# Griffan/VerifyBamID

Measured on AMD Instinct MI355X. Metric: llk_evals_per_sec, higher is better.
Workload: dtype f64; 1 GPU; synthetic pileup 100000 markers x depth 30, --NumPC 4 (BASELINE.json configs[2] shape); parallelism=1 GPU, rccl_world_size=1, launched_by=single process, reads=2999230, active_markers=100000, distinct_codes=42, device=gfx950:sramecc+:xnack-

## Files before the change

### verifybamid_amd/csrc/kernel_debug.h

```cpp
#ifndef VB2_KERNEL_DEBUG_H_
#define VB2_KERNEL_DEBUG_H_

#ifndef VB2_ABLATE
#define VB2_ABLATE 0
#endif
#ifndef VB2_FLAG_RELEASE
#define VB2_FLAG_RELEASE 1
#endif
#ifndef VB2_SOFT_PROLOGUE
#define VB2_SOFT_PROLOGUE 1
#endif
#ifndef VB2_CTRL_PRIO
#define VB2_CTRL_PRIO 3
#endif
#ifndef VB2_SPLIT_FAST
#define VB2_SPLIT_FAST 3
#endif
#ifndef VB2_STAMP_ROUND
#define VB2_STAMP_ROUND 0
#endif

namespace vb2 {
constexpr int kAblNoMap = 1, kAblNoTable = 2, kAblNoItems = 4, kAblNoReads = 8, kAblNoEpi = 16, kAblNoSignal = 32, kAblNoMul = 64, kAblNoRowLoads = 128;
constexpr int kAblate = VB2_ABLATE;
constexpr int kSplitFast = VB2_SPLIT_FAST;
}

#ifdef VB2_WITH_STAMPS
#define VB2_STAMPS_OF(L) ((L).stamps)
#else
#define VB2_STAMPS_OF(L) (static_cast<unsigned long long*>(nullptr))
#endif

#ifdef VB2_ITEM_PROF
#define VB2_IP_T(var) const unsigned long long var = __builtin_readcyclecounter()
#define VB2_IP_USE(x) asm volatile("" ::"v"(x))
#else
#define VB2_IP_T(var)
#define VB2_IP_USE(x)
#endif

#endif
```

### verifybamid_amd/csrc/llk_kernels.hip

```cpp
#include "llk_kernels.h"

#include <hip/hip_runtime.h>
#include <link.h>

#include "kernel_debug.h"
#include "tile_sched.h"
#include "tunables.h"
#ifndef VB2_SIMD_DEAL
#define VB2_SIMD_DEAL 1
#endif

#include <algorithm>
#include <atomic>
#include <cstring>
#include <type_traits>
#include <vector>

namespace vb2 {

__device__ __forceinline__ void pair_of(int p, int& g1, int& g2)
{
    g1 = p >> 1;
    const int lo = p & 1;
    g2 = lo + (lo >= g1 ? 1 : 0);
// ... 247 lines not shown
}
__device__ __forceinline__ int lane_of(int m, int g)
{
    const int idx = ((g & 1) << 2) + (m >> 2);
    const int q = (0x74216530u >> (4 * idx)) & 7;
    return ((g >> 1) << 5) + (q << 2) + (m & 3);
}

__device__ __forceinline__ int lane_xchg_i32(int x, int off, int partner)
{
    if (off == 1) return __builtin_amdgcn_update_dpp(0, x, 0xB1, 0xf, 0xf, true);
    if (off == 2) return __builtin_amdgcn_update_dpp(0, x, 0x4E, 0xf, 0xf, true);
    if (off == 4) {
        const int a = __builtin_amdgcn_update_dpp(0, x, 0x124, 0xf, 0x5, false);
        return __builtin_amdgcn_update_dpp(a, x, 0x12C, 0xf, 0xa, false);
    }
    return __shfl(x, partner, 64);
}
__device__ __forceinline__ double lane_xchg_f64(double x, int off, int partner)
{
    if (off == 1 || off == 2 || off == 4)
        return __hiloint2double(lane_xchg_i32(__double2hiint(x), off, partner), lane_xchg_i32(__double2loint(x), off, partner));
    return __shfl(x, partner, 64);
}

template <int MODE> struct Geom { static constexpr int kMaxWaves = 16, kBlocksPerCU = 1, kWavesPerSimd = 4; };
template <int MODE> struct ModeNp { static constexpr int value = MODE == 2 ? 8 : MODE == 4 ? 1 : MODE == 5 ? 2 : 4; };

struct InlinePoints {
    int count;
    double v[kInlinePointDoubles];
};

struct NoHook {
    __device__ bool on_block() const { return false; }
    __device__ bool mine() const { return false; }
    __device__ void run() {}
    __device__ bool keep_etab() const { return false; }
    __device__ bool prim_in_lds() const { return false; }
    __device__ bool keep_prim() const { return false; }
    __device__ double* sum_stage() const { return nullptr; }
    __device__ uint32_t cache_rec() const { return 0u; }
    __device__ unsigned int* sync_word() const { return nullptr; }
    __device__ bool collect_only() const { return false; }
    __device__ bool no_collect() const { return false; }
};
__host__ __device__ __forceinline__ bool eval_is_dynamic(const DeviceLayout& L, uint32_t nblk, int nwave, int ngrp)
{
    const uint32_t max_tiles_blk = owned_most(L.pd ? 1 : 0, (uint32_t)L.num_mt, nblk);
    return max_tiles_blk * (uint32_t)ngrp <= (uint32_t)(L.dyn_limit * nwave);
}

template <int MODE, bool W16 = false, class Hook = NoHook, bool STREAM = false, int QUEUE = -1, int KSEL = 0,
          bool LCACHE = false, int ESH = 8, bool PD = false, int SPLIT = 0>
__device__ __forceinline__ void
eval_body(const DeviceLayout& L, const double* ip_v, const int ip_count, const double* __restrict__ points, int num_valid,
          double* __restrict__ partials, double* __restrict__ llk_out,
          unsigned int* __restrict__ ticket, unsigned long long* __restrict__ done_flag,
          unsigned long long done_seq, const uint32_t blk, const uint32_t nblk,
          unsigned int* __restrict__ batch_done, unsigned int batch_active, const int ngrp_in,
          const unsigned long long tag, const Schedule sch, const bool coherent_points = false,
          const int tid_in = -1, const double* lds_rows = nullptr ,
          Hook hook = Hook())
{
    extern __shared__ __attribute__((aligned(16))) double lds[];
    static_assert(MODE >= 2 && MODE <= 5, "wave shapes 2..5");
    static_assert(!PD || ESH == 8, "probability-domain contexts have no exp table");
    static_assert(!(PD && W16) || ((MODE == 4 || MODE == 5) && STREAM), "8-bit step lists: cohort steps of one and two points");
    static_assert(!SPLIT || (PD && MODE == 2 && QUEUE == 1 && !STREAM && !LCACHE), "split launches: the 8-point shape on the queue");
    constexpr int OSH = PD ? 1 : 0;
    constexpr bool ONEGRP = MODE != 2 || STREAM;
    constexpr int KAF = KSEL > 0 ? 0 : -1;
    constexpr int BTL = MODE == 4 ? 1 : 2;
    constexpr int TPW = MODE == 3 ? 2 : (MODE == 4 || MODE == 5) ? 4 : 1;
    constexpr int SLOTS = 4 / TPW;
    constexpr int NP = SLOTS * BTL;
    const int row_bytes = MODE == 2 ? kRowBytesWide : L.row_bytes;
    const int RS = row_bytes >> 3;
    const int nrow = L.num_code + 1;
    const int nthread = blockDim.x;
    const int nwave = nthread >> 6;
    const int k = KSEL > 0 ? KSEL : L.num_pc;
    const int stride = 2 * k + 1;
    constexpr int NVS = SPLIT ? SPLIT : 1;
    const int g_per = SPLIT ? (ngrp_in + NVS - 1) / NVS : ngrp_in;
    const int g_lo = SPLIT ? (int)(blk % (uint32_t)NVS) * g_per : 0;
    const int ngrp = ONEGRP ? 1 : SPLIT ? (ngrp_in - g_lo < g_per ? ngrp_in - g_lo : g_per) : ngrp_in;
    const int p_off = g_lo * NP;
    const uint32_t vstep = SPLIT ? nblk / (uint32_t)NVS : 0u, vb0 = SPLIT ? blk / (uint32_t)NVS : blk;
    const double* const known_af_p = KAF == 0 ? nullptr : L.known_af;
    const int NPT = NP * ngrp;
    constexpr int kEtabCopies = (1 << ESH) / 8, kEtabDoubles = PD ? 0 : 64 * kEtabCopies;
    constexpr int kLtabDoubles = PD ? 0 : kLogTabDoubles;
    double* etab = lds;
    double* ltab = lds + kEtabDoubles;
    double* tab = ltab + kLtabDoubles;
    double* red = tab + ngrp * nrow * RS;
    unsigned int* queue = reinterpret_cast<unsigned int*>(red + NVS * NPT);
    double* pts = red + NVS * NPT + 2;
    double* ptq = pts + (size_t)NPT * stride + ((NPT * stride) & 1);
    const size_t prim_off = (size_t)(ptq - lds) + (size_t)NPT * 2 * k;
    double2* prim_lds = reinterpret_cast<double2*>(lds + prim_off + (prim_off & 1));
    double* tile_llk = reinterpret_cast<double*>(prim_lds + L.num_prim);

    const int tid = tid_in >= 0 ? tid_in : (int)threadIdx.x;
    const int lane = tid & 63;
    const int wave = __builtin_amdgcn_readfirstlane(tid >> 6);
    int m, g4;
    lane_map(lane, m, g4);
    const int g = g4 & (SLOTS - 1);
    const int half = TPW == 1 ? 0 : g4 / SLOTS;
    const bool stamp_this = VB2_STAMP_ROUND == 0 || (unsigned)(tag & 0xffffffffull) == (unsigned)VB2_STAMP_ROUND;
#ifdef VB2_ITEM_PROF
    unsigned long long* stamps = nullptr;
#else
    unsigned long long* stamps = (VB2_STAMPS_OF(L) && stamp_this) ? VB2_STAMPS_OF(L) + (size_t)blk * 8 : nullptr;
#endif
    if (stamps && tid == 0) { stamps[0] = wall_clock64(); stamps[4] = 0; }
    if constexpr (SPLIT != 0) {
        if (stamps && tid == 0 && blk != 0u && blk != 20u && blk != 21u) {
            unsigned int xcc;
            asm volatile("s_getreg_b32 %0, hwreg(HW_REG_XCC_ID)" : "=s"(xcc));
            stamps[7] = 1ull + (xcc & 15u);
        }
    }

    const bool collect_only = hook.collect_only();
    if (collect_only && hook.mine()) hook.run();
    if (!collect_only) {
    const bool hook_blk = hook.on_block(), hook_mine = hook.mine();
    unsigned int* const soft_word = PD ? hook.sync_word() : nullptr;
    const bool soft = hook_blk && soft_word != nullptr;
    if (soft && hook_mine) hook.run();
    const int ptid = !soft ? tid : hook_mine ? 0x3fffffff : tid - 64, pnthread = soft ? nthread - 64 : nthread;
    unsigned int soft_gen = 0;
    auto prologue_sync = [&]() {
        if (!soft) { __syncthreads(); return; }
        if (hook_mine) return;
        soft_gen += (unsigned int)(nwave - 1);
        if (lane == 0) __hip_atomic_fetch_add(soft_word, 1u, __ATOMIC_RELAXED, __HIP_MEMORY_SCOPE_WORKGROUP);
        while (__hip_atomic_load(soft_word, __ATOMIC_RELAXED, __HIP_MEMORY_SCOPE_WORKGROUP) < soft_gen) __builtin_amdgcn_s_sleep(1);
        asm volatile("" ::: "memory");
    };
    constexpr bool SPLIT_EARLY = SPLIT != 0 && (kSplitFast & 1) != 0;
    constexpr int kTabSide = 3;
    const int ntab_split = (kAblate & kAblNoTable) ? 0 : (PD ? L.num_prim - L.num_pair : L.num_prim) * 6 * NP;
    auto table_inputs = [&](int e, int g0, double2& rec_o, double* al_o) {
        const int pi = e / (6 * NP);
        const int bb = (e - pi * (6 * NP)) / 6;
        rec_o = L.prim[pi];
#pragma unroll
        for (int u = 0; u < kTabSide; ++u) {
            const int ge = g0 + u < ngrp ? g0 + u : ngrp - 1;
            const int b = ge * NP + bb;
            const int idx = (p_off + b < num_valid ? p_off + b : num_valid - 1) * stride + 2 * k;
            al_o[u] = (kAblate & kAblNoMap) ? 0.01 * (double)(1 + idx % 7) : points[idx];
        }
    };
    double2 tin_rec = make_double2(0.0, 0.0);
    double tin_al[kTabSide] = {0.0, 0.0, 0.0};
    if constexpr (SPLIT_EARLY)
        if (ptid < ntab_split) table_inputs(ptid, 0, tin_rec, tin_al);
    if (ptid == 0) *queue = (unsigned int)(nwave - (hook_blk ? 1 : 0));
    for (int e = ptid; e < NPT * stride; e += pnthread) {
        const int b = e / stride;
        const int src = p_off + b < num_valid ? p_off + b : num_valid - 1;
        const int idx = src * stride + (e - b * stride);
        const double v = (kAblate & kAblNoMap) ? 0.01 * (double)(1 + idx % 7)
                         : lds_rows ? lds_rows[idx]
                         : ip_count > 0 ? ip_v[idx]
                         : coherent_points ? __hip_atomic_load(&points[idx], __ATOMIC_RELAXED, __HIP_MEMORY_SCOPE_AGENT)
                                           : points[idx];
        pts[e] = v;
        const int c = e - b * stride;
        if (c < 2 * k) ptq[((b / BTL) * 2 * k + c) * BTL + (b % BTL)] = v;
    }
    if (!PD && !hook.keep_etab() && tid < kLogTabDoubles / 2)
        reinterpret_cast<double2*>(ltab)[tid] = kLogTabRows[tid];
    if (!PD && !hook.keep_etab())
        for (int jb = 2 * wave; jb < 64; jb += 2 * nwave) {
            const double t0 = kExp2Tab[jb], t1 = kExp2Tab[jb + 1];
            const double tv = lane < 32 ? exp_tab_entry(t0, jb) : exp_tab_entry(t1, jb + 1);
            if constexpr (ESH == 8) etab[jb * 32 + lane] = tv;
            else if ((lane & 31) < kEtabCopies) etab[(jb + (lane >> 5)) * kEtabCopies + (lane & 31)] = tv;
        }
    const bool prim_kept = hook.prim_in_lds() && hook.keep_prim();
    const bool staged = ngrp > 1 || (hook.prim_in_lds() && !prim_kept) || (PD && L.num_pair > 0 && !prim_kept);
    if (staged)
        for (int e = ptid; e < L.num_prim; e += pnthread) prim_lds[e] = L.prim[e];
    const bool early_table = lds_rows != nullptr && !staged;
    if (!early_table && !SPLIT_EARLY) prologue_sync();
    if (stamps && (soft ? ptid : tid) == 0) stamps[1] = wall_clock64();

    const uint32_t ltab_addr = lds_byte_addr(ltab);
    const int num_single = PD ? L.num_prim - L.num_pair : L.num_prim;
    if constexpr (SPLIT_EARLY) {
        int e = ptid, g0 = 0;
        while (e < ntab_split) {
            int e_n = e, g0_n = g0 + kTabSide;
            if (g0_n >= ngrp) {
                g0_n = 0;
                e_n = e + pnthread;
            }
            double2 rec_n = tin_rec;
            double al_n[kTabSide] = {tin_al[0], tin_al[1], tin_al[2]};
            if (e_n < ntab_split) table_inputs(e_n, g0_n, rec_n, al_n);
            const int pi = e / (6 * NP);
            const int bp = e - pi * (6 * NP);
            const int bb = bp / 6, p = bp - bb * 6;
            (void)bb;
            const uint32_t pr = (uint32_t)__double_as_longlong(tin_rec.y);
            const int dc = (int)(pr & 0xffffu), twin = (int)(pr >> 16);
            int g1, g2;
            pair_of(p, g1, g2);
            double v3[kTabSide], r3[kTabSide];
            double* cell3[kTabSide];
#pragma unroll
            for (int u = 0; u < kTabSide; ++u) {
                const int ge = g0 + u < ngrp ? g0 + u : ngrp - 1;
                v3[u] = prob_entry(tin_al[u], tin_rec.x, g1, g2);
                r3[u] = v3[u];
                cell3[u] = tab + (size_t)ge * nrow * RS + dc * RS + bp;
                *cell3[u] = r3[u];
            }
            const int kq = twin & 0xff, pstride = RS * (int)(int8_t)(twin >> 8);
            for (int n = 1; n < kq; ++n) {
#pragma unroll
                for (int u = 0; u < kTabSide; ++u) {
                    r3[u] *= v3[u];
                    cell3[u] += pstride;
                    *cell3[u] = r3[u];
                }
            }
            tin_rec = rec_n;
#pragma unroll
            for (int u = 0; u < kTabSide; ++u) tin_al[u] = al_n[u];
            e = e_n;
            g0 = g0_n;
        }
    } else
    for (int e = ptid; e < ((kAblate & kAblNoTable) ? 0 : num_single * 6 * NP); e += pnthread) {
        const int pi = e / (6 * NP);
        const int bp = e - pi * (6 * NP);
        const int bb = bp / 6, p = bp - bb * 6;
        const double2 rec = (staged || prim_kept) ? prim_lds[pi] : L.prim[pi];
        const uint32_t pr = (uint32_t)__double_as_longlong(rec.y);
        const int dc = (int)(pr & 0xffffu), twin = (int)(pr >> 16);
        int g1, g2;
// ... 2 lines not shown
            constexpr int kSide = 3;
            for (int g0 = 0; g0 < ngrp; g0 += kSide) {
                double v3[kSide], r3[kSide];
                double* cell3[kSide];
#pragma unroll
                for (int u = 0; u < kSide; ++u) {
                    const int ge = g0 + u < ngrp ? g0 + u : ngrp - 1;
                    v3[u] = prob_entry(pts[(ge * NP + bb) * stride + 2 * k], rec.x, g1, g2);
                    r3[u] = v3[u];
                    cell3[u] = tab + (size_t)ge * nrow * RS + dc * RS + bp;
                    *cell3[u] = r3[u];
                }
                const int kq = twin & 0xff, pstride = RS * (int)(int8_t)(twin >> 8);
                for (int n = 1; n < kq; ++n) {
#pragma unroll
                    for (int u = 0; u < kSide; ++u) {
                        r3[u] *= v3[u];
                        cell3[u] += pstride;
                        *cell3[u] = r3[u];
                    }
                }
            }
        } else
#pragma clang loop unroll(disable)
        for (int grp_e = 0; grp_e < ngrp; ++grp_e) {
            const double alpha_e = early_table ? lds_rows[(bb < num_valid ? bb : num_valid - 1) * stride + 2 * k]
                                               : pts[(grp_e * NP + bb) * stride + 2 * k];
            double* gtab = tab + (size_t)grp_e * nrow * RS;
            if constexpr (PD) {
                const double v = prob_entry(alpha_e, rec.x, g1, g2);
                double r = v;
                double* cell = gtab + dc * RS + bp;
                constexpr int kMir = kPdAltOffset / 8;
                const int mir = kMir + bb * 6 + (5 - p) - bp;
                *cell = r;
                if constexpr (NP <= 4 && STREAM) cell[mir] = r;
                const int kq = twin & 0xff, pstride = RS * (int)(int8_t)(twin >> 8);
                for (int n = 1; n < kq; ++n) {
                    r *= v;
                    cell += pstride;
                    *cell = r;
                    if constexpr (NP <= 4 && STREAM) cell[mir] = r;
                }
            } else {
                const double v = table_entry(alpha_e, rec.x, g1, g2, ltab_addr);
                const double tv = W16 ? 0.5 * v : v;
                gtab[dc * RS + bp] = tv;
                if (twin != 0xffff) gtab[twin * RS + bb * 6 + (5 - p)] = tv;
            }
        }
    }
    for (int e = ptid; e < ngrp * RS; e += pnthread) {
        const int grp_e = e / RS;
        tab[((size_t)grp_e * nrow + L.num_code) * RS + (e - grp_e * RS)] = PD ? 1.0 : 0.0;
    }
    if constexpr (PD) {
        for (int level = 0; level < 2 && L.num_pair > 0 && !(kAblate & kAblNoTable); ++level) {
            const int nrec = level == 0 ? L.num_pair - L.num_pair2 : L.num_pair2;
            if (nrec == 0) break;
            prologue_sync();
            const double2* const prec = prim_lds + num_single + (level == 0 ? 0 : L.num_pair - L.num_pair2);
            for (int e = ptid; e < nrec * 6 * NP; e += pnthread) {
                const int pi = e / (6 * NP);
                const int bp = e - pi * (6 * NP);
                const double2 rec = prec[pi];
                const uint32_t ab = (uint32_t)__double_as_longlong(rec.x), dst = (uint32_t)__double_as_longlong(rec.y);
                const int ra = (int)(ab & 0xffffu) * RS + bp, rb = (int)(ab >> 16) * RS + bp, rd = (int)dst * RS + bp;
                constexpr int kMir = kPdAltOffset / 8;
                const int bb = bp / 6, p = bp - bb * 6;
                const int mir = kMir + bb * 6 + (5 - p) - bp;
#pragma clang loop unroll(disable)
                for (int grp_e = 0; grp_e < ngrp; ++grp_e) {
                    double* gtab = tab + (size_t)grp_e * nrow * RS;
                    const double v = gtab[ra] * gtab[rb];
                    gtab[rd] = v;
                    if constexpr (NP <= 4 && STREAM) gtab[rd + mir] = v;
                }
            }
        }
    }
    prologue_sync();
    if (stamps && (soft ? ptid : tid) == 0) stamps[2] = wall_clock64();

    const uint32_t nt_v0 = owned_count(OSH, (uint32_t)L.num_mt, vb0, nblk);
    const uint32_t nt_v1 = SPLIT ? owned_count(OSH, (uint32_t)L.num_mt, vb0 + vstep, nblk) : 0u;
    const uint32_t nt_v2 = SPLIT > 2 ? owned_count(OSH, (uint32_t)L.num_mt, vb0 + 2u * vstep, nblk) : 0u;
    auto nt_of = [&](uint32_t vs) { return vs == 0u ? nt_v0 : vs == 1u ? nt_v1 : nt_v2; };
    const uint32_t ntile_blk = nt_v0;
    const size_t mp = L.m_pad;
    const uint32_t nunit = SPLIT ? (uint32_t)NVS * ntile_blk : (ntile_blk + TPW - 1) / TPW;
    const uint32_t nitem = (kAblate & kAblNoItems) ? 0u : nunit * (uint32_t)ngrp;
    const float inv_nunit = 1.0f / (float)(nunit ? nunit : 1u);
    const uint32_t ngrp_magic = ngrp > 1 ? 0xFFFFFFFFu / (uint32_t)ngrp + 1u : 0u;
    const bool dyn = QUEUE < 0 ? eval_is_dynamic(L, nblk, nwave, ngrp) : QUEUE != 0;
    typedef unsigned int __attribute__((ext_vector_type(2))) vuint2;
    typedef __attribute__((address_space(1))) const vuint2 g_cuint2;
    typedef __attribute__((address_space(1))) const double g_cdouble;
    typedef __attribute__((address_space(1))) const char g_cchar;
    g_cuint2* const g_rec = (g_cuint2*)(W16 ? L.mt_rec16 : L.mt_rec);
    g_cuint2* const g_codes = (g_cuint2*)(W16 ? L.codes16 : L.codes);
    typedef __attribute__((address_space(1))) const uint32_t g_cuint;
    typedef __attribute__((address_space(3))) const uint32_t lds_cuint;
    typedef typename std::conditional<PD, uint32_t, vuint2>::type RowWord;
    constexpr uint32_t kRowBytes = PD ? kMtMarkers * 4u : kMtMarkers * 8u, kLaneBytes = PD ? 4u : 8u;
    g_cdouble* const g_ediag = (g_cdouble*)L.ediag;
    g_cdouble* const g_ud = (g_cdouble*)L.ud;
    g_cdouble* const g_mu = (g_cdouble*)L.mu;
    g_cdouble* const g_kaf = (g_cdouble*)known_af_p;
    auto tile_product = [&](ScaledProd* p, bool cross) {
#pragma unroll
        for (int off = 8; off >= 1; off >>= 1) {
            const int partner = lane_of(m ^ off, g4);
#pragma unroll
            for (int t = 0; t < BTL; ++t) {
                p[t].m *= lane_xchg_f64(p[t].m, off, partner);
                p[t].e += lane_xchg_f64(p[t].e, off, partner);
            }
        }
        if (!cross) return;
#pragma unroll
        for (int off = SLOTS; off < 4; off <<= 1) {
            const int partner = lane_of(m, g4 ^ off);
#pragma unroll
            for (int t = 0; t < BTL; ++t) {
                p[t].m *= __shfl(p[t].m, partner, 64);
                p[t].e += __shfl(p[t].e, partner, 64);
            }
        }
    };
    LaneProd wave_prod[BTL];
#pragma unroll
    for (int t = 0; t < BTL; ++t) wave_prod[t] = LaneProd{1.0, 0};
    int nfactor = 0;
    auto renorm_wave = [&]() {
#pragma unroll
        for (int t = 0; t < BTL; ++t) {
            wave_prod[t].e += __builtin_amdgcn_frexp_exp(wave_prod[t].m);
            wave_prod[t].m = __builtin_amdgcn_frexp_mant(wave_prod[t].m);
        }
// ... 43 lines not shown
    };
    auto tile_of = [&](uint32_t idx_, bool& have_) -> uint32_t {
        const uint32_t it_ = TPW * idx_ + (uint32_t)half;
        have_ = idx_ < nitem && (TPW == 1 || it_ < ntile_blk);
        return have_ ? owned_tile(OSH, blk, nblk, it_) : owned_tile(OSH, blk, nblk, 0u);
    };
    auto draw_item = [&]() -> uint32_t {
        uint32_t nxt = 0;
        if (lane == 0) nxt = atomicAdd(queue, 1u);
        return (uint32_t)__builtin_amdgcn_readfirstlane(nxt);
    };
    auto issue_rows = [&](const vuint2 rec_, bool have_) {
        const uint32_t cb_ = rec_.x * kRowBytes + (uint32_t)m * kLaneBytes;
        const int rows_ = have_ ? (PD ? (int)(((rec_.y >> 16) + (W16 ? 3u : 1u)) >> (W16 ? 2 : 1)) : (int)rec_.y) : 0;
        const int last_ = rows_ > 0 ? rows_ - 1 : 0;
#pragma unroll
        for (int j = 0; j < kPf; ++j) {
            g_cchar* a_ = reinterpret_cast<g_cchar*>(g_codes) + (cb_ + (uint32_t)(j < last_ ? j : last_) * kRowBytes);
            if constexpr (PD) w[j] = *reinterpret_cast<g_cuint*>(a_);
            else w[j] = *reinterpret_cast<g_cuint2*>(a_);
        }
    };
    auto walk_word = [&](const vuint2 w_cur, double* acc, const uint32_t my_tab, const uint32_t my_tab_w16, auto first_tag,
                         const double init) {
        constexpr bool kFirst = decltype(first_tag)::value;
        if constexpr ((kAblate & kAblNoReads) != 0) {
            acc[0] += __hiloint2double((int)((w_cur.x ^ w_cur.y) & 0x000f0000u) | 0x3ff00000, 0);
            return;
        }
#pragma unroll
        for (int j = 0; j < (W16 ? 4 : 2); ++j) {
            double n;
            uint32_t row_addr;
            if constexpr (W16) {
                const uint32_t w2 = (j & 2) ? w_cur.y : w_cur.x;
                const uint32_t idx = (j & 1) ? ((w2 >> 16) & 0xffu) : (w2 & 0xffu);
                const uint32_t hi = __builtin_amdgcn_perm(0x40000000u, w2, (j & 1) ? 0x07030c0cu : 0x07010c0cu);
                n = __hiloint2double((int)hi, 0);
                row_addr = my_tab_w16 + __umul24(idx, (uint32_t)row_bytes);
            } else {
                const uint32_t rw = j ? w_cur.y : w_cur.x;
                n = __hiloint2double((int)(rw & 0xffff0000u), 0);
                row_addr = my_tab + (rw & 0xffffu);
            }
            lds_cdouble2* row = reinterpret_cast<lds_cdouble2*>(row_addr);
#pragma unroll
            for (int i = 0; i < 3 * BTL; ++i) {
                const vdouble2 t = row[i];
                acc[2 * i] = fma(n, t.x, (kFirst && j == 0) ? init : acc[2 * i]);
                acc[2 * i + 1] = fma(n, t.y, (kFirst && j == 0) ? init : acc[2 * i + 1]);
            }
        }
    };
    auto walk_pd = [&](const uint32_t w_cur, double* acc, const uint32_t my_tab, auto alt0_tag, auto alt1_tag, auto first_tag) {
        constexpr bool kAlt0 = decltype(alt0_tag)::value, kAlt1 = decltype(alt1_tag)::value, kFirst = decltype(first_tag)::value;
        if constexpr ((kAblate & kAblNoReads) != 0) {
            acc[0] = (kFirst ? 1.0 : acc[0]) * __hiloint2double((int)((w_cur ^ (w_cur >> 16)) & 0x000fu) | 0x3ff00000, 0);
            return;
        }
#pragma unroll
        for (int j = 0; j < 2; ++j) {
            const bool kAlt = j ? kAlt1 : kAlt0;
            const uint32_t row_addr = (kAlt ? my_tab - (uint32_t)kPdAltOffset : my_tab) + (j ? (w_cur >> 16) : (w_cur & 0xffffu));
            lds_cdouble2* row = reinterpret_cast<lds_cdouble2*>(row_addr);
#pragma unroll
            for (int i = 0; i < 3 * BTL; ++i) {
                const vdouble2 t = row[i];
                const int pt = i / 3, q2 = 2 * (i - 3 * pt);
                const int a0 = pt * 6 + (kAlt ? 5 - q2 : q2), a1 = pt * 6 + (kAlt ? 4 - q2 : q2 + 1);
                if constexpr ((kAblate & kAblNoMul) != 0) {
                    asm volatile("" ::"v"(t.x), "v"(t.y));
                    if (kFirst && j == 0) { acc[a0] = t.x; acc[a1] = t.y; }
                    continue;
                }
                acc[a0] = (kFirst && j == 0) ? t.x : acc[a0] * t.x;
                acc[a1] = (kFirst && j == 0) ? t.y : acc[a1] * t.y;
            }
        }
    };
    auto walk_pd1 = [&](const uint32_t w_cur, double* acc, const uint32_t my_tab, auto first_tag) {
        constexpr bool kFirst = decltype(first_tag)::value;
#pragma unroll
        for (int j = 0; j < 2; ++j) {
            const uint32_t row_addr = my_tab + (j ? (w_cur >> 16) : (w_cur & 0xffffu));
            lds_cdouble2* row = reinterpret_cast<lds_cdouble2*>(row_addr);
#pragma unroll
            for (int i = 0; i < 3 * BTL; ++i) {
                const vdouble2 t = row[i];
                acc[2 * i] = (kFirst && j == 0) ? t.x : acc[2 * i] * t.x;
                acc[2 * i + 1] = (kFirst && j == 0) ? t.y : acc[2 * i + 1] * t.y;
            }
        }
    };
    auto walk_pd8 = [&](const uint32_t w_cur, double* acc, const uint32_t my_tab, auto first_tag, const int step0, const int s1) {
        constexpr bool kFirst = decltype(first_tag)::value;
#pragma unroll
        for (int j = 0; j < 4; ++j) {
            const uint32_t idx = (w_cur >> (8 * j)) & 0xffu;
            const uint32_t base = (step0 + j >= s1) ? my_tab + (uint32_t)kPdAltOffset : my_tab;
            const uint32_t row_addr = base + __umul24(idx, (uint32_t)row_bytes);
            lds_cdouble2* row = reinterpret_cast<lds_cdouble2*>(row_addr);
#pragma unroll
            for (int i = 0; i < 3 * BTL; ++i) {
                const vdouble2 t = row[i];
                acc[2 * i] = (kFirst && j == 0) ? t.x : acc[2 * i] * t.x;
                acc[2 * i + 1] = (kFirst && j == 0) ? t.y : acc[2 * i + 1] * t.y;
            }
        }
    };
    auto marker_lk = [&](const bool live, const uint32_t pos, const double* acc, const double e0, const double e1, const double e2,
                         const double* udr, const double mur, const uint32_t my_ptq, double* lk_m, int* lk_e, const double cst_pd) {
#pragma unroll
        for (int t = 0; t < BTL; ++t) { lk_m[t] = 1.0; lk_e[t] = 0; }
        if constexpr ((kAblate & kAblNoEpi) != 0) {
            double z = e0 + e1 + e2 + mur + udr[0] + udr[1] + udr[2] + udr[3];
            for (int i = 0; i < BTL * 6; ++i) z += acc[i];
            if (z == 12345.678) lk_m[0] = 0.75;
            return;
        }
        if (live) {
            double af1[BTL], af2[BTL];
            if (known_af_p) {
                const double a = g_kaf[pos];
#pragma unroll
                for (int t = 0; t < BTL; ++t) af1[t] = af2[t] = a;
            } else {
#pragma unroll
                for (int t = 0; t < BTL; ++t) af1[t] = af2[t] = 0.;
                auto project = [&](int kk, double uu) {
                    if constexpr (BTL == 2) {
                        const vdouble2 c1 = *reinterpret_cast<lds_cdouble2*>(my_ptq + (uint32_t)kk * 16u);
                        const vdouble2 c2 = *reinterpret_cast<lds_cdouble2*>(my_ptq + (uint32_t)(k + kk) * 16u);
                        af1[0] = fma(uu, c1.x, af1[0]); af1[1] = fma(uu, c1.y, af1[1]);
                        af2[0] = fma(uu, c2.x, af2[0]); af2[1] = fma(uu, c2.y, af2[1]);
                    } else {
                        af1[0] = fma(uu, *reinterpret_cast<lds_cdouble*>(my_ptq + (uint32_t)kk * 8u), af1[0]);
                        af2[0] = fma(uu, *reinterpret_cast<lds_cdouble*>(my_ptq + (uint32_t)(k + kk) * 8u), af2[0]);
                    }
                };
#pragma unroll
                for (int kk = 0; kk < 4; ++kk)
                    if (kk < k) project(kk, udr[kk]);
                for (int kk = 4; kk < k; ++kk) project(kk, g_ud[(size_t)kk * mp + pos]);
                const double mu = mur;
#pragma unroll
                for (int t = 0; t < BTL; ++t) {
                    af1[t] += mu; af1[t] /= 2.0;
                    af2[t] += mu; af2[t] /= 2.0;
                }
            }
#pragma unroll
            for (int t = 0; t < BTL; ++t) {
                double gf[3], gf2[3];
                initial_gf(af1[t], gf);
                initial_gf(af2[t], gf2);
                const double* a = acc + t * 6;
                double x01, x02, x10, x12, x20, x21;
                const double a_min = PD ? 0.0 : vmin2_f64(vmin2_f64(vmin2_f64(a[0], a[1]), vmin2_f64(a[2], a[3])), vmin2_f64(a[4], a[5]));
                if constexpr (PD) {
                    x01 = a[0]; x02 = a[1]; x10 = a[2]; x12 = a[3]; x20 = a[4]; x21 = a[5];
                } else
                if (__builtin_expect(a_min < -708.0, 0)) {
                    x01 = exp_nonpos<ESH, true>(a[0], etab_lane); x02 = exp_nonpos<ESH, true>(a[1], etab_lane);
                    x10 = exp_nonpos<ESH, true>(a[2], etab_lane); x12 = exp_nonpos<ESH, true>(a[3], etab_lane);
                    x20 = exp_nonpos<ESH, true>(a[4], etab_lane); x21 = exp_nonpos<ESH, true>(a[5], etab_lane);
                } else {
                    x01 = exp_nonpos<ESH>(a[0], etab_lane); x02 = exp_nonpos<ESH>(a[1], etab_lane);
                    x10 = exp_nonpos<ESH>(a[2], etab_lane); x12 = exp_nonpos<ESH>(a[3], etab_lane);
                    x20 = exp_nonpos<ESH>(a[4], etab_lane); x21 = exp_nonpos<ESH>(a[5], etab_lane);
                }
                double lk;
                if constexpr (PD) {
                    const double o0 = fma(x02, gf2[2], x01 * gf2[1]);
                    const double o1 = fma(x12, gf2[2], x10 * gf2[0]);
                    const double o2 = fma(x21, gf2[1], x20 * gf2[0]);
                    const double off = fma(o2, gf[2], fma(o1, gf[1], o0 * gf[0]));
                    const double dg = fma(e2 * gf2[2], gf[2], fma(e1 * gf2[1], gf[1], (e0 * gf2[0]) * gf[0]));
                    lk = fma(cst_pd, off, dg);
                    if (__builtin_expect(lk < 0x1p-960, 0)) {
                        x01 *= cst_pd; x02 *= cst_pd; x10 *= cst_pd; x12 *= cst_pd; x20 *= cst_pd; x21 *= cst_pd;
                    }
                } else {
                const double s0 = fma(x02, gf2[2], fma(x01, gf2[1], e0 * gf2[0]));
                const double s1 = fma(x12, gf2[2], fma(e1, gf2[1], x10 * gf2[0]));
                const double s2 = fma(e2, gf2[2], fma(x21, gf2[1], x20 * gf2[0]));
// ... 146 lines not shown
                if constexpr (PD) return *reinterpret_cast<g_cuint*>(a_);
                else return *reinterpret_cast<g_cuint2*>(a_);
            }
        };
        if (!PIPE) {
#pragma unroll
            for (int j = 0; j < kPf; ++j) w[j] = load_row(j);
        }
        auto walk_block = [&](const int s0, const bool refill, auto first_tag) {
            constexpr bool kFirstBlock = decltype(first_tag)::value;
#pragma unroll
            for (int u = 0; u < kPf; ++u) {
                if (s0 + u >= rows) break;
                const RowWord w_cur = w[u];
                if (refill) w[u] = load_row(s0 + u + kPf);
                if constexpr (PD) {
                    if constexpr (W16) {
                        if (kFirstBlock && u == 0) walk_pd8(w_cur, acc, my_tab, std::true_type(), (s0 + u) * 4, steps_ref);
                        else walk_pd8(w_cur, acc, my_tab, std::false_type(), (s0 + u) * 4, steps_ref);
                    } else {
                        if (kFirstBlock && u == 0) walk_pd1(w_cur, acc, my_tab, std::true_type());
                        else walk_pd1(w_cur, acc, my_tab, std::false_type());
                    }
                } else {
                    if (kFirstBlock && u == 0) walk_word(w_cur, acc, my_tab, my_tab_w16, std::true_type(), cst);
                    else walk_word(w_cur, acc, my_tab, my_tab_w16, std::false_type(), cst);
                }
            }
        };
        VB2_IP_USE(w[0].x);
        VB2_IP_T(ip_t2);
        if constexpr (PD && TPW > 1 && STREAM) {
            if (__any(rows == 0)) {
                if (rows == 0) {
#pragma unroll
                    for (int i = 0; i < BTL * 6; ++i) acc[i] = 1.0;
                }
            }
            if constexpr (PIPE) {
                const bool more = __any(rows > kPf);
                walk_block(0, more, std::true_type());
                if (more)
                    for (int s0 = kPf; s0 < rows; s0 += kPf) walk_block(s0, true, std::false_type());
                issue_rows(rec_n2, have_next);
                cst_nx = other_const(mt_next, have_next);
                rec_nx = rec_n2;
            } else {
                walk_block(0, true, std::true_type());
                for (int s0 = kPf; s0 < rows; s0 += kPf) walk_block(s0, true, std::false_type());
            }
        } else if constexpr (PD) {
            int r = 0;
            static_assert(kPf == 2, "the ring below has two slots");
            auto row_step = [&](auto slot_tag, auto alt0_tag, auto alt1_tag, auto first_tag) {
                constexpr int kSlot = decltype(slot_tag)::value;
                const uint32_t cur = w[kSlot];
                w[kSlot] = load_row(r + kPf);
                walk_pd(cur, acc, my_tab, alt0_tag, alt1_tag, first_tag);
                ++r;
            };
            const std::integral_constant<int, 0> kS0;
            const std::integral_constant<int, 1> kS1;
            const int rows_ra = steps_ref >> 1;
            const std::false_type kRef;
            const std::true_type kAltT, kFirstT;
            const std::false_type kNotFirst;
            if (rows > 0) {
                if (steps_ref >= 2) row_step(kS0, kRef, kRef, kFirstT);
                else if (steps_ref == 1) row_step(kS0, kRef, kAltT, kFirstT);
                else row_step(kS0, kAltT, kAltT, kFirstT);
            } else {
#pragma unroll
                for (int i = 0; i < BTL * 6; ++i) acc[i] = 1.0;
            }
            auto rows_of_kind = [&](const int end, auto alt_tag) {
                if (r < end && (r & 1)) row_step(kS1, alt_tag, alt_tag, kNotFirst);
                while (r + 1 < end) {
                    row_step(kS0, alt_tag, alt_tag, kNotFirst);
                    row_step(kS1, alt_tag, alt_tag, kNotFirst);
                }
                if (r < end) row_step(kS0, alt_tag, alt_tag, kNotFirst);
            };
            rows_of_kind(rows_ra, kRef);
            if ((steps_ref & 1) && r == rows_ra && r < rows) {
                if (r & 1) row_step(kS1, kRef, kAltT, kNotFirst);
                else row_step(kS0, kRef, kAltT, kNotFirst);
            }
            rows_of_kind(rows, kAltT);
            if constexpr (PIPE) {
                issue_rows(rec_n2, have_next);
                cst_nx = other_const(mt_next, have_next);
                rec_nx = rec_n2;
            }
        } else if constexpr (PIPE) {
            const bool more = __any(rows > kPf);
            walk_block(0, more, std::false_type());
            if (more)
                for (int s0 = kPf; s0 < rows; s0 += kPf) walk_block(s0, true, std::false_type());
            issue_rows(rec_n2, have_next);
            cst_nx = other_const(mt_next, have_next);
            rec_nx = rec_n2;
        } else if constexpr (PEEL) {
            if (rows > 0) {
                walk_block(0, true, std::true_type());
                for (int s0 = kPf; s0 < rows; s0 += kPf) walk_block(s0, true, std::false_type());
            } else {
#pragma unroll
                for (int i = 0; i < BTL * 6; ++i) acc[i] = cst;
            }
        } else {
            for (int s0 = 0; s0 < rows; s0 += kPf) walk_block(s0, true, std::false_type());
        }

        __builtin_amdgcn_s_setprio(0);
#ifdef VB2_STAMP_CTRL
        if (stamps && lane == 0 && wave == 1 && !hook_blk) stamps[3] = wall_clock64();
#else
        if (stamps && lane == 0 && wave == 1) stamps[3] = wall_clock64();
#endif
        VB2_IP_USE(acc[0]); VB2_IP_USE(acc[BTL * 6 - 1]);
        VB2_IP_T(ip_t3);
        VB2_IP_USE(e0); VB2_IP_USE(e1); VB2_IP_USE(e2); VB2_IP_USE(mur); VB2_IP_USE(udr[0]); VB2_IP_USE(udr[3]);
        VB2_IP_T(ip_t4);
        double lk_m[BTL];
        int lk_e[BTL];
        marker_lk(live, pos, acc, e0, e1, e2, udr, mur, my_ptq, lk_m, lk_e, cst);
        VB2_IP_USE(lk_m[0]); VB2_IP_USE(lk_m[BTL - 1]);
        VB2_IP_T(ip_t5);
        if (!dyn) {
#pragma unroll
            for (int t = 0; t < BTL; ++t) {
                wave_prod[t].m *= lk_m[t];
                wave_prod[t].e += lk_e[t];
            }
            if (++nfactor == kLazyRenorm) renorm_wave();
            if (have_sched) {
                ++s_i;
                idx = PIPE ? idx_next : (s_i < s_end ? (uint32_t)sch.item[s_i] : nitem);
                continue;
            }
            ++round;
// ... 201 lines not shown
                    for (int w = 0; w < NPT; ++w) stage[(size_t)w * nb + b] = __builtin_nan("");
                    break;
                }
                __builtin_amdgcn_s_sleep(1);
            }
        }
    }
    __syncthreads();
    for (int b = wave; b < num_valid; b += nwave) {
        const double* p = stage + (size_t)b * nb;
        double s = 0;
        for (int base = 0; base < nb; base += 8 * 64) {
            double x[8];
#pragma unroll
            for (int q = 0; q < 8; ++q) {
                const int i = base + q * 64 + lane;
                x[q] = i < nb ? p[i] : 0.0;
            }
#pragma unroll
            for (int q = 0; q < 8; ++q) s += x[q];
        }
        s = wave_sum(s);
        if (lane == 0) put_result(b, s);
    }
    }
    if (VB2_STAMPS_OF(L) && tid == 0) {
        const unsigned long long t6 = wall_clock64();
        if (stamps) stamps[6] = t6;
        if ((collect_only || (blk == 0 && !hook.no_collect())) && nblk > 32) VB2_STAMPS_OF(L)[21 * 8 + 7] += t6 - VB2_STAMPS_OF(L)[7];
    }
    if (done_flag && !(kAblate & kAblNoSignal)) {
        asm volatile("s_waitcnt vmcnt(0)" ::: "memory");
        __syncthreads();
        if (tid == 0) {
            bool signal = true;
            if (batch_done) {
                const unsigned int t = __hip_atomic_fetch_add(batch_done, 1u, __ATOMIC_RELAXED, __HIP_MEMORY_SCOPE_AGENT);
                signal = (t == batch_active - 1);
                if (signal) __hip_atomic_store(batch_done, 0u, __ATOMIC_RELAXED, __HIP_MEMORY_SCOPE_AGENT);
            }
            if (signal)
                __hip_atomic_store(done_flag, done_seq, VB2_FLAG_RELEASE ? __ATOMIC_RELEASE : __ATOMIC_RELAXED, __HIP_MEMORY_SCOPE_SYSTEM);
        }
    }
}

template <int MODE, int QUEUE, int KSEL = 0, bool PD = false>
__global__ void __launch_bounds__(Geom<MODE>::kMaxWaves * 64, Geom<MODE>::kWavesPerSimd)
llk_eval_kernel(const DeviceLayout L, const InlinePoints ip, const double* __restrict__ points,
                int num_valid, double* __restrict__ partials, double* __restrict__ llk_out,
                unsigned int* __restrict__ ticket, unsigned long long* __restrict__ done_flag,
                unsigned long long done_seq, int ngrp, unsigned long long tag, const Schedule sch)
{
    eval_body<MODE, false, NoHook, false, QUEUE, KSEL, false, 8, PD>(L, ip.v, ip.count, points, num_valid, partials, llk_out, ticket,
                                                                     done_flag, done_seq, blockIdx.x, gridDim.x, nullptr, 0u, ngrp, tag, sch);
}

template <int KSEL, int S>
__global__ void __launch_bounds__(Geom<2>::kMaxWaves * 64, Geom<2>::kWavesPerSimd)
llk_eval_split_kernel(const DeviceLayout L, const double* __restrict__ points, int num_valid, double* __restrict__ partials,
                      double* __restrict__ llk_out, unsigned int* __restrict__ ticket, unsigned long long* __restrict__ done_flag,
                      unsigned long long done_seq, int ngrp)
{
    eval_body<2, false, NoHook, false, 1, KSEL, false, 8, true, S>(L, nullptr, 0, points, num_valid, partials, llk_out, ticket, done_flag,
                                                                     done_seq, blockIdx.x, gridDim.x, nullptr, 0u, ngrp, 0ull,
                                                                     Schedule{nullptr, nullptr});
}

template <int KSEL, bool PD = false>
__global__ void __launch_bounds__(Geom<2>::kMaxWaves * 64, Geom<2>::kWavesPerSimd)
llk_eval_passes_kernel(const DeviceLayout L, const double* __restrict__ points, int num_valid, int points_per_pass,
                       double* __restrict__ partials, double* __restrict__ llk_out, unsigned int* __restrict__ tickets,
                       unsigned long long* __restrict__ done_flag, unsigned long long done_seq,
                       unsigned long long* __restrict__ scratch_flag)
{
    const int stride = 2 * L.num_pc + 1;
    int pass = 0;
    for (int first = 0; first < num_valid; first += points_per_pass, ++pass) {
        const int left = num_valid - first;
        const int nv = left < points_per_pass ? left : points_per_pass;
        const bool last = left <= points_per_pass;
        if (pass > 0) __syncthreads();
        eval_body<2, false, NoHook, false, 1, KSEL, false, (PD ? 8 : 6), PD>(
            L, nullptr, 0, points + (size_t)first * stride, nv, partials + (size_t)first * gridDim.x, llk_out + first,
            tickets + pass, (last || !done_flag) ? done_flag : scratch_flag, done_seq, blockIdx.x, gridDim.x, nullptr, 0u,
            (nv + 7) / 8, 0ull, Schedule{nullptr, nullptr});
    }
}

#define VB2_PASSES_KERNEL_ARGS                                                                                           \
    const DeviceLayout, const double*, int, int, double*, double*, unsigned int*, unsigned long long*, unsigned long long, \
        unsigned long long*
#if defined(VB2_TU_MAIN)
extern template __global__ void llk_eval_passes_kernel<4>(VB2_PASSES_KERNEL_ARGS);
extern template __global__ void llk_eval_passes_kernel<2>(VB2_PASSES_KERNEL_ARGS);
extern template __global__ void llk_eval_passes_kernel<0>(VB2_PASSES_KERNEL_ARGS);
extern template __global__ void llk_eval_passes_kernel<4, true>(VB2_PASSES_KERNEL_ARGS);
extern template __global__ void llk_eval_passes_kernel<2, true>(VB2_PASSES_KERNEL_ARGS);
extern template __global__ void llk_eval_passes_kernel<0, true>(VB2_PASSES_KERNEL_ARGS);
#elif defined(VB2_TU_PASSES)
template __global__ void llk_eval_passes_kernel<4>(VB2_PASSES_KERNEL_ARGS);
template __global__ void llk_eval_passes_kernel<2>(VB2_PASSES_KERNEL_ARGS);
template __global__ void llk_eval_passes_kernel<0>(VB2_PASSES_KERNEL_ARGS);
template __global__ void llk_eval_passes_kernel<4, true>(VB2_PASSES_KERNEL_ARGS);
template __global__ void llk_eval_passes_kernel<2, true>(VB2_PASSES_KERNEL_ARGS);
template __global__ void llk_eval_passes_kernel<0, true>(VB2_PASSES_KERNEL_ARGS);
#endif

template <int MODE, bool W16, int KSEL = 0, int STATIC = 0, bool PD = false>
__global__ void __launch_bounds__(Geom<MODE>::kMaxWaves * 64, Geom<MODE>::kWavesPerSimd)
llk_eval_multi_kernel(const DeviceLayout* __restrict__ layouts, const Schedule* __restrict__ scheds,
                      const double* __restrict__ points,
                      const int* __restrict__ num_valid, double* __restrict__ partials,
                      double* __restrict__ llk_out, unsigned int* __restrict__ tickets, int bps,
                      unsigned long long* __restrict__ done_flag, unsigned long long done_seq,
                      unsigned int* __restrict__ batch_done, unsigned int batch_active, int use_ticket,
                      const MultiInline mi)
// ... 602 lines not shown
```

### verifybamid_amd/csrc/resident_kernel.inc

```
__device__ __forceinline__ double* lds_base()
{
    extern __shared__ __attribute__((aligned(16))) double lds[];
    return lds;
}

__device__ const unsigned long long kLibmExpTab[256] = {
#include "libm_exp_table.inc"
};

__device__ __forceinline__ double libm_exp(double x, const __attribute__((address_space(3))) unsigned long long* tab )
{
    const double InvLn2N = 0x1.71547652b82fep0 * 128, NegLn2hiN = -0x1.62e42fefa0000p-8,
                 NegLn2loN = -0x1.cf79abc9e3b3ap-47, Shift = 0x1.8p52;
    const double C2 = 0x1.ffffffffffdbdp-2, C3 = 0x1.555555555543cp-3, C4 = 0x1.55555cf172b91p-5,
                 C5 = 0x1.1111167a4d017p-7;
    double kd = fma(InvLn2N, x, Shift);
    const unsigned long long ki = (unsigned long long)__double_as_longlong(kd);
    kd -= Shift;
    const double r = fma(kd, NegLn2loN, fma(kd, NegLn2hiN, x));
    const unsigned idx = 2u * (unsigned)(ki & 127u);
    const double tail = __longlong_as_double((long long)tab[idx]);
    const unsigned long long sbits = tab[idx + 1] + (ki << 45);
    const double r2 = r * r;
    const double tmp = fma(r2 * r2, fma(r, C5, C4), fma(r2, fma(r, C3, C2), tail + r));
// ... 1120 lines not shown
        const unsigned long long got = stage_hdr[0];
        if (got == ~0ull || (got >> 16) != round) {
            if (ctl_blk && tid == 0)
                __hip_atomic_store(ra.h_state, 3u, __ATOMIC_RELAXED, __HIP_MEMORY_SCOPE_SYSTEM);
            return;
        }
        const int code = (int)(got & 0xff);
        if (code == (int)kRelayEmptyRound) continue;
        const int nv = code;
        if (nv <= 0) {
            if (ctl_blk && tid == 0)
                __hip_atomic_store(ra.h_state, 2u, __ATOMIC_RELAXED, __HIP_MEMORY_SCOPE_SYSTEM);
            return;
        }
        const double* lds_rows = lds_base() + stage_hdr[1];
        if (VB2_STAMPS_OF(L) && ctl_blk && tid == 0) {
            const unsigned long long t_has = wall_clock64();
            VB2_STAMPS_OF(L)[7] = t_has;
            if (prof && shared[0] != 0) {
                VB2_STAMPS_OF(L)[8 + 7] += t_ctl - t_top;
                VB2_STAMPS_OF(L)[16 + 7] += t_has - t_ctl;
                VB2_STAMPS_OF(L)[32 + 7] += 1;
            }
        }
        const bool search_round = ctl_blk && shared[0] != 0;
        double* dst = search_round ? DeviceSimplex::ycand_of(sx_base) : ra.h_out;
        unsigned long long* dflag = search_round ? nullptr : ra.h_done;
        const unsigned long long dseq = ctl_blk ? shared[1] : 0ull;
        const unsigned long long tag = (ra.epoch << 32) | round;
        DeviceLayout Lr = L;
        asm volatile("" : "+s"(Lr.codes), "+s"(Lr.mt_rec), "+s"(Lr.ud), "+s"(Lr.mu), "+s"(Lr.ediag),
                          "+s"(Lr.known_af), "+s"(Lr.prim));
        asm volatile("" : "+s"(Lr.num_code), "+s"(Lr.row_bytes), "+s"(Lr.num_prim), "+s"(Lr.num_mt),
                          "+s"(Lr.num_pc), "+s"(Lr.num_active), "+s"(Lr.m_pad), "+s"(Lr.dyn_limit));
        int tid_r = tid;
        asm volatile("" : "+v"(tid_r));
        ControlHook hook;
        hook.blk = search_round && may_speculate;
        hook.me = hook.blk && wave == 0;
        hook.st = st;
        hook.spec = ra.spec;
        hook.round = round;
        hook.nmax = ra.state_nmax;
        hook.k = k;
        hook.lane = lane;
        hook.prof = prof_ctl;
        hook.etab_ok = etab_built && (!ctl_blk || sum_stage != nullptr);
        hook.only_collects = extra_ctl && ctl_blk;
        hook.collects_elsewhere = extra_ctl && !ctl_blk;
        etab_built = true;
        hook.stage_sums = sum_stage;
        hook.crec = crec_addr;
        hook.sync = VB2_SOFT_PROLOGUE ? reinterpret_cast<unsigned int*>(stage + 2) : nullptr;
        eval_body<3, false, ControlHook, false, QUEUE, KSEL, LCACHE, 8, PD>(Lr, nullptr, 0, nullptr, nv, partials, dst, ticket, dflag, dseq, blockIdx.x,
                                                   nblk_eval, nullptr, 0u, 1, tag, ra.sched_multi, false, tid_r, lds_rows,
                                                   hook);
    }
}
```

Baseline: 1.041 million evals/s.

## Issue both read-row LDS loads before multiplies in probability-domain walk

Adds a per-kernel-family reads-ahead mode to the probability-domain read walk. Both table rows for a packed read pair are loaded from LDS before the multiplies run, with scheduling barriers to group loads ahead of FMAs. An optional mode also prefetches the epilogue projection coefficients during the final read step. Separately, layout sizes are pinned in scalar registers for one non-PD kernel variant. This aims to hide LDS latency in the inner read loop, at the cost of more VGPRs for the staged rows, which may reduce occupancy.

```diff
diff --git a/verifybamid_amd/csrc/kernel_debug.h b/verifybamid_amd/csrc/kernel_debug.h
--- a/verifybamid_amd/csrc/kernel_debug.h
+++ b/verifybamid_amd/csrc/kernel_debug.h
@@ -16,6 +16,9 @@
 #ifndef VB2_SPLIT_FAST
 #define VB2_SPLIT_FAST 3
 #endif
+#ifndef VB2_READS_AHEAD
+#define VB2_READS_AHEAD 0x0111
+#endif
 #ifndef VB2_STAMP_ROUND
 #define VB2_STAMP_ROUND 0
 #endif
@@ -24,6 +27,8 @@
 constexpr int kAblNoMap = 1, kAblNoTable = 2, kAblNoItems = 4, kAblNoReads = 8, kAblNoEpi = 16, kAblNoSignal = 32, kAblNoMul = 64, kAblNoRowLoads = 128;
 constexpr int kAblate = VB2_ABLATE;
 constexpr int kSplitFast = VB2_SPLIT_FAST;
+constexpr int kReadsAheadMask = VB2_READS_AHEAD;
+constexpr int reads_ahead(int family) { return (kReadsAheadMask >> (4 * family)) & 0xf; }
 }
 
 #ifdef VB2_WITH_STAMPS
diff --git a/verifybamid_amd/csrc/llk_kernels.hip b/verifybamid_amd/csrc/llk_kernels.hip
--- a/verifybamid_amd/csrc/llk_kernels.hip
+++ b/verifybamid_amd/csrc/llk_kernels.hip
@@ -323,7 +323,7 @@
 }
 
 template <int MODE, bool W16 = false, class Hook = NoHook, bool STREAM = false, int QUEUE = -1, int KSEL = 0,
-          bool LCACHE = false, int ESH = 8, bool PD = false, int SPLIT = 0>
+          bool LCACHE = false, int ESH = 8, bool PD = false, int SPLIT = 0, int RAHEAD = 0>
 __device__ __forceinline__ void
 eval_body(const DeviceLayout& L, const double* ip_v, const int ip_count, const double* __restrict__ points, int num_valid,
           double* __restrict__ partials, double* __restrict__ llk_out,
@@ -346,9 +346,20 @@
     constexpr int TPW = MODE == 3 ? 2 : (MODE == 4 || MODE == 5) ? 4 : 1;
     constexpr int SLOTS = 4 / TPW;
     constexpr int NP = SLOTS * BTL;
-    const int row_bytes = MODE == 2 ? kRowBytesWide : L.row_bytes;
+    constexpr int kReadsAhead = PD ? RAHEAD : 0;
+    constexpr bool kOwnSizes = QUEUE == 0 && KSEL == 0 && !PD && !STREAM && (MODE == 3 || MODE == 4) && std::is_same<Hook, NoHook>::value;
+    int own_num_code = 0, own_row_bytes = 0, own_num_prim = 0, own_num_mt = 0;
+    if constexpr (kOwnSizes) {
+        own_num_code = L.num_code; own_row_bytes = L.row_bytes; own_num_prim = L.num_prim; own_num_mt = L.num_mt;
+        asm volatile("" : "+s"(own_num_code), "+s"(own_row_bytes), "+s"(own_num_prim), "+s"(own_num_mt));
+    }
+    const auto l_num_code = [&] { if constexpr (kOwnSizes) return own_num_code; else return L.num_code; };
+    const auto l_row_bytes = [&] { if constexpr (kOwnSizes) return own_row_bytes; else return L.row_bytes; };
+    const auto l_num_prim = [&] { if constexpr (kOwnSizes) return own_num_prim; else return L.num_prim; };
+    const auto l_num_mt = [&] { if constexpr (kOwnSizes) return own_num_mt; else return L.num_mt; };
+    const int row_bytes = MODE == 2 ? kRowBytesWide : l_row_bytes();
     const int RS = row_bytes >> 3;
-    const int nrow = L.num_code + 1;
+    const int nrow = l_num_code() + 1;
     const int nthread = blockDim.x;
     const int nwave = nthread >> 6;
     const int k = KSEL > 0 ? KSEL : L.num_pc;
@@ -372,7 +383,7 @@
     double* ptq = pts + (size_t)NPT * stride + ((NPT * stride) & 1);
     const size_t prim_off = (size_t)(ptq - lds) + (size_t)NPT * 2 * k;
     double2* prim_lds = reinterpret_cast<double2*>(lds + prim_off + (prim_off & 1));
-    double* tile_llk = reinterpret_cast<double*>(prim_lds + L.num_prim);
+    double* tile_llk = reinterpret_cast<double*>(prim_lds + l_num_prim());
 
     const int tid = tid_in >= 0 ? tid_in : (int)threadIdx.x;
     const int lane = tid & 63;
@@ -415,7 +426,7 @@
     };
     constexpr bool SPLIT_EARLY = SPLIT != 0 && (kSplitFast & 1) != 0;
     constexpr int kTabSide = 3;
-    const int ntab_split = (kAblate & kAblNoTable) ? 0 : (PD ? L.num_prim - L.num_pair : L.num_prim) * 6 * NP;
+    const int ntab_split = (kAblate & kAblNoTable) ? 0 : (PD ? l_num_prim() - L.num_pair : l_num_prim()) * 6 * NP;
     auto table_inputs = [&](int e, int g0, double2& rec_o, double* al_o) {
         const int pi = e / (6 * NP);
         const int bb = (e - pi * (6 * NP)) / 6;
@@ -458,13 +469,13 @@
     const bool prim_kept = hook.prim_in_lds() && hook.keep_prim();
     const bool staged = ngrp > 1 || (hook.prim_in_lds() && !prim_kept) || (PD && L.num_pair > 0 && !prim_kept);
     if (staged)
-        for (int e = ptid; e < L.num_prim; e += pnthread) prim_lds[e] = L.prim[e];
+        for (int e = ptid; e < l_num_prim(); e += pnthread) prim_lds[e] = L.prim[e];
     const bool early_table = lds_rows != nullptr && !staged;
     if (!early_table && !SPLIT_EARLY) prologue_sync();
     if (stamps && (soft ? ptid : tid) == 0) stamps[1] = wall_clock64();
 
     const uint32_t ltab_addr = lds_byte_addr(ltab);
-    const int num_single = PD ? L.num_prim - L.num_pair : L.num_prim;
+    const int num_single = PD ? l_num_prim() - L.num_pair : l_num_prim();
     if constexpr (SPLIT_EARLY) {
         int e = ptid, g0 = 0;
         while (e < ntab_split) {
@@ -573,7 +584,7 @@
     }
     for (int e = ptid; e < ngrp * RS; e += pnthread) {
         const int grp_e = e / RS;
-        tab[((size_t)grp_e * nrow + L.num_code) * RS + (e - grp_e * RS)] = PD ? 1.0 : 0.0;
+        tab[((size_t)grp_e * nrow + l_num_code()) * RS + (e - grp_e * RS)] = PD ? 1.0 : 0.0;
     }
     if constexpr (PD) {
         for (int level = 0; level < 2 && L.num_pair > 0 && !(kAblate & kAblNoTable); ++level) {
@@ -603,9 +614,9 @@
     prologue_sync();
     if (stamps && (soft ? ptid : tid) == 0) stamps[2] = wall_clock64();
 
-    const uint32_t nt_v0 = owned_count(OSH, (uint32_t)L.num_mt, vb0, nblk);
-    const uint32_t nt_v1 = SPLIT ? owned_count(OSH, (uint32_t)L.num_mt, vb0 + vstep, nblk) : 0u;
-    const uint32_t nt_v2 = SPLIT > 2 ? owned_count(OSH, (uint32_t)L.num_mt, vb0 + 2u * vstep, nblk) : 0u;
+    const uint32_t nt_v0 = owned_count(OSH, (uint32_t)l_num_mt(), vb0, nblk);
+    const uint32_t nt_v1 = SPLIT ? owned_count(OSH, (uint32_t)l_num_mt(), vb0 + vstep, nblk) : 0u;
+    const uint32_t nt_v2 = SPLIT > 2 ? owned_count(OSH, (uint32_t)l_num_mt(), vb0 + 2u * vstep, nblk) : 0u;
     auto nt_of = [&](uint32_t vs) { return vs == 0u ? nt_v0 : vs == 1u ? nt_v1 : nt_v2; };
     const uint32_t ntile_blk = nt_v0;
     const size_t mp = L.m_pad;
@@ -755,10 +766,57 @@
             }
         }
     };
-    auto walk_pd = [&](const uint32_t w_cur, double* acc, const uint32_t my_tab, auto alt0_tag, auto alt1_tag, auto first_tag) {
+    constexpr bool kEpiAhead = (kReadsAhead == 3 || kReadsAhead == 4) && KSEL > 0 && BTL == 2;
+    constexpr int kCqK = !kEpiAhead ? 0 : (kReadsAhead == 3 || KSEL < 2) ? KSEL : 2;
+    constexpr int kCq = kEpiAhead ? 2 * kCqK : 1;
+    vdouble2 cq[kCq];
+    uint32_t cq_addr = 0;
+    auto request_cq = [&]() {
+#pragma unroll
+        for (int i = 0; i < kCq; ++i) cq[i] = *reinterpret_cast<lds_cdouble2*>(cq_addr + (uint32_t)((i & 1) * KSEL + (i >> 1)) * 16u);
+    };
+    auto walk_pd = [&](const uint32_t w_cur, double* acc, const uint32_t my_tab, auto alt0_tag, auto alt1_tag, auto first_tag, auto pre_tag) {
         constexpr bool kAlt0 = decltype(alt0_tag)::value, kAlt1 = decltype(alt1_tag)::value, kFirst = decltype(first_tag)::value;
+        constexpr bool kPre = decltype(pre_tag)::value;
         if constexpr ((kAblate & kAblNoReads) != 0) {
             acc[0] = (kFirst ? 1.0 : acc[0]) * __hiloint2double((int)((w_cur ^ (w_cur >> 16)) & 0x000fu) | 0x3ff00000, 0);
+            return;
+        }
+        if constexpr (kReadsAhead != 0 && !kFirst && (kAblate & kAblNoMul) == 0) {
+            vdouble2 t[6 * BTL];
+            auto request = [&](const int j) {
+                const bool kAlt = j ? kAlt1 : kAlt0;
+                const uint32_t row_addr = (kAlt ? my_tab - (uint32_t)kPdAltOffset : my_tab) + (j ? (w_cur >> 16) : (w_cur & 0xffffu));
+                lds_cdouble2* row = reinterpret_cast<lds_cdouble2*>(row_addr);
+#pragma unroll
+                for (int i = 0; i < 3 * BTL; ++i) t[j * 3 * BTL + i] = row[i];
+            };
+            auto multiply = [&](const int j) {
+                const bool kAlt = j ? kAlt1 : kAlt0;
+#pragma unroll
+                for (int i = 0; i < 3 * BTL; ++i) {
+                    const int pt = i / 3, q2 = 2 * (i - 3 * pt);
+                    const int a0 = pt * 6 + (kAlt ? 5 - q2 : q2), a1 = pt * 6 + (kAlt ? 4 - q2 : q2 + 1);
+                    acc[a0] = acc[a0] * t[j * 3 * BTL + i].x;
+                    acc[a1] = acc[a1] * t[j * 3 * BTL + i].y;
+                }
+            };
+            if constexpr (kReadsAhead == 1 || kReadsAhead == 3 || kReadsAhead == 4) {
+                request(0); request(1);
+                if constexpr (kPre) request_cq();
+                multiply(0); multiply(1);
+                __builtin_amdgcn_sched_group_barrier(0x100, 6 * BTL + (kPre ? kCq : 0), 0);
+                __builtin_amdgcn_sched_group_barrier(0x002, 12 * BTL, 0);
+            } else {
+#pragma unroll
+                for (int j = 0; j < 2; ++j) {
+                    request(j);
+                    multiply(j);
+                    __builtin_amdgcn_sched_group_barrier(0x100, 3 * BTL, 0);
+                    __builtin_amdgcn_sched_group_barrier(0x002, 6 * BTL, 0);
+                    __builtin_amdgcn_sched_barrier(0);
+                }
+            }
             return;
         }
 #pragma unroll
@@ -832,8 +890,12 @@
                 for (int t = 0; t < BTL; ++t) af1[t] = af2[t] = 0.;
                 auto project = [&](int kk, double uu) {
                     if constexpr (BTL == 2) {
-                        const vdouble2 c1 = *reinterpret_cast<lds_cdouble2*>(my_ptq + (uint32_t)kk * 16u);
-                        const vdouble2 c2 = *reinterpret_cast<lds_cdouble2*>(my_ptq + (uint32_t)(k + kk) * 16u);
+                        vdouble2 c1, c2;
+                        if (kEpiAhead && kk < kCqK) { c1 = cq[kCq > 1 ? 2 * kk : 0]; c2 = cq[kCq > 1 ? 2 * kk + 1 : 0]; }
+                        else {
+                            c1 = *reinterpret_cast<lds_cdouble2*>(my_ptq + (uint32_t)kk * 16u);
+                            c2 = *reinterpret_cast<lds_cdouble2*>(my_ptq + (uint32_t)(k + kk) * 16u);
+                        }
                         af1[0] = fma(uu, c1.x, af1[0]); af1[1] = fma(uu, c1.y, af1[1]);
                         af2[0] = fma(uu, c2.x, af2[0]); af2[1] = fma(uu, c2.y, af2[1]);
                     } else {
@@ -1086,12 +1148,15 @@
         } else if constexpr (PD) {
             int r = 0;
             static_assert(kPf == 2, "the ring below has two slots");
-            auto row_step = [&](auto slot_tag, auto alt0_tag, auto alt1_tag, auto first_tag) {
+            auto row_step_pre = [&](auto slot_tag, auto alt0_tag, auto alt1_tag, auto first_tag, auto pre_tag) {
                 constexpr int kSlot = decltype(slot_tag)::value;
                 const uint32_t cur = w[kSlot];
                 w[kSlot] = load_row(r + kPf);
-                walk_pd(cur, acc, my_tab, alt0_tag, alt1_tag, first_tag);
+                walk_pd(cur, acc, my_tab, alt0_tag, alt1_tag, first_tag, pre_tag);
                 ++r;
+            };
+            auto row_step = [&](auto slot_tag, auto alt0_tag, auto alt1_tag, auto first_tag) {
+                row_step_pre(slot_tag, alt0_tag, alt1_tag, first_tag, std::false_type());
             };
             const std::integral_constant<int, 0> kS0;
             const std::integral_constant<int, 1> kS1;
@@ -1115,12 +1180,37 @@
                 }
                 if (r < end) row_step(kS0, alt_tag, alt_tag, kNotFirst);
             };
+            if constexpr (kEpiAhead) {
+                cq_addr = my_ptq;
+                const int last = rows - 1;
+                rows_of_kind(rows_ra < last ? rows_ra : last, kRef);
+                if ((steps_ref & 1) && r == rows_ra && r < last) {
+                    if (r & 1) row_step(kS1, kRef, kAltT, kNotFirst);
+                    else row_step(kS0, kRef, kAltT, kNotFirst);
+                }
+                rows_of_kind(last, kAltT);
+                const std::true_type kPreT;
+                if (r < rows) {
+                    if (r < rows_ra) {
+                        if (r & 1) row_step_pre(kS1, kRef, kRef, kNotFirst, kPreT);
+                        else row_step_pre(kS0, kRef, kRef, kNotFirst, kPreT);
+                    } else if ((steps_ref & 1) && r == rows_ra) {
+                        if (r & 1) row_step_pre(kS1, kRef, kAltT, kNotFirst, kPreT);
+                        else row_step_pre(kS0, kRef, kAltT, kNotFirst, kPreT);
+                    } else {
+                        if (r & 1) row_step_pre(kS1, kAltT, kAltT, kNotFirst, kPreT);
+                        else row_step_pre(kS0, kAltT, kAltT, kNotFirst, kPreT);
+                    }
+                } else
+                    request_cq();
+            } else {
             rows_of_kind(rows_ra, kRef);
             if ((steps_ref & 1) && r == rows_ra && r < rows) {
                 if (r & 1) row_step(kS1, kRef, kAltT, kNotFirst);
                 else row_step(kS0, kRef, kAltT, kNotFirst);
             }
             rows_of_kind(rows, kAltT);
+            }
             if constexpr (PIPE) {
                 issue_rows(rec_n2, have_next);
                 cst_nx = other_const(mt_next, have_next);
@@ -1428,7 +1518,7 @@
                 unsigned int* __restrict__ ticket, unsigned long long* __restrict__ done_flag,
                 unsigned long long done_seq, int ngrp, unsigned long long tag, const Schedule sch)
 {
-    eval_body<MODE, false, NoHook, false, QUEUE, KSEL, false, 8, PD>(L, ip.v, ip.count, points, num_valid, partials, llk_out, ticket,
+    eval_body<MODE, false, NoHook, false, QUEUE, KSEL, false, 8, PD, 0, reads_ahead(MODE == 2 ? 1 : 2)>(L, ip.v, ip.count, points, num_valid, partials, llk_out, ticket,
                                                                      done_flag, done_seq, blockIdx.x, gridDim.x, nullptr, 0u, ngrp, tag, sch);
 }
 
@@ -1438,7 +1528,7 @@
                       double* __restrict__ llk_out, unsigned int* __restrict__ ticket, unsigned long long* __restrict__ done_flag,
                       unsigned long long done_seq, int ngrp)
 {
-    eval_body<2, false, NoHook, false, 1, KSEL, false, 8, true, S>(L, nullptr, 0, points, num_valid, partials, llk_out, ticket, done_flag,
+    eval_body<2, false, NoHook, false, 1, KSEL, false, 8, true, S, reads_ahead(0)>(L, nullptr, 0, points, num_valid, partials, llk_out, ticket, done_flag,
                                                                      done_seq, blockIdx.x, gridDim.x, nullptr, 0u, ngrp, 0ull,
                                                                      Schedule{nullptr, nullptr});
 }
diff --git a/verifybamid_amd/csrc/resident_kernel.inc b/verifybamid_amd/csrc/resident_kernel.inc
--- a/verifybamid_amd/csrc/resident_kernel.inc
+++ b/verifybamid_amd/csrc/resident_kernel.inc
@@ -1196,7 +1196,7 @@
         hook.stage_sums = sum_stage;
         hook.crec = crec_addr;
         hook.sync = VB2_SOFT_PROLOGUE ? reinterpret_cast<unsigned int*>(stage + 2) : nullptr;
-        eval_body<3, false, ControlHook, false, QUEUE, KSEL, LCACHE, 8, PD>(Lr, nullptr, 0, nullptr, nv, partials, dst, ticket, dflag, dseq, blockIdx.x,
+        eval_body<3, false, ControlHook, false, QUEUE, KSEL, LCACHE, 8, PD, 0, reads_ahead(3)>(Lr, nullptr, 0, nullptr, nv, partials, dst, ticket, dflag, dseq, blockIdx.x,
                                                    nblk_eval, nullptr, 0u, 1, tag, ra.sched_multi, false, tid_r, lds_rows,
                                                    hook);
     }
```

New measurement: 1.060 million evals/s (median of 6 runs). +1.8%, better.
